# tashoyan/locations-recommender

Measured on AMD Instinct MI355X. Metric: KNN person-pair cosines/s (cosine place+category, combine, top-K), higher is better.
Workload: dtype u16 dot (exact, packed) / f64 cosine

## Files before the change

### locations-recommender_amd/csrc/knn.hip

```cpp

#include <algorithm>
#include <chrono>
#include <cstring>
#include <cmath>
#include <cstdlib>
#include <memory>
#include <new>
#include <numeric>
#include <type_traits>
#include <unordered_map>

#include "knn_index.h"

namespace {

using namespace locrec;

constexpr uint32_t kEmpty = 0xFFFFFFFFu;
constexpr int kMergeCap = 8192;
constexpr int kAggCap = 4096;
constexpr int kDirectMaxBytes = cfg::kDirectMaxBytes;
constexpr int kLdsSoftLimit = 64 * 1024;
constexpr int kLdsHardLimit = 160 * 1024;

// ... 406 lines not shown
    p.mode = 3;
    p.qt = ht.qt;
    p.waves = ht.waves;
    p.S = std::max(64, pow2ceil(2 * K));
    auto fam = [&](const DevFamily &d, const DevBuf<uint32_t> &sell, const DevBuf<int64_t> &off, const DevBuf<int32_t> &w,
                   Family &f) {
        f = Family{};
        f.sell = sell.p;
        f.sell_off = off.p;
        f.sell_w = w.p;
        f.norm = d.norm.p;
        f.inorm32 = d.inorm32.p;
        f.csr_ptr = d.csr_ptr.p;
        f.csr_idx = d.csr_idx.p;
        f.csr_val = d.csr_val.p;
        f.direct = 1;
    };
    fam(ix->fp, ht.p_sell, ht.p_off, ht.p_w, p.fp);
    fam(ix->fc, ht.c_sell, ht.c_off, ht.c_w, p.fc);
    p.fp.rows_cap = ht.h;
    p.fc.rows_cap = ix->fc.dim;
    size_t cur = (size_t)kHtCatRows * p.qt * 2 + (size_t)cfg::ht_plane_rows(ht.h) * p.qt * 2;
    cur = (cur + 15) & ~(size_t)15;
    p.off_tail = (int)cur;
    cur += (size_t)p.waves * 64 * p.qt * 2;
    p.off_cand_s = (int)cur;
    cur += (size_t)p.qt * p.S * sizeof(double);
    p.off_cand_rid = (int)cur;
    cur += (size_t)p.qt * p.S * sizeof(uint32_t);
    cur = (cur + 15) & ~(size_t)15;
    p.off_misc = (int)cur;
    cur += (size_t)p.qt * (3 * sizeof(double) + 8 * sizeof(int32_t)) + 16;
    cur = (cur + 15) & ~(size_t)15;
    p.off_queue = (int)cur;
    cur += (size_t)p.waves * kQueueCap * 16 + (size_t)p.waves * 4 + 16;
    p.lds = cur;
    if (cur > (size_t)kLdsHardLimit) return false;
    pl = p;
    return true;
}

int32_t enqueue_ht_prepass(locrec_knn_index *ix, const int32_t *qrows_dev, int32_t qrow0, int64_t nq, int qt,
                           int64_t total_hits)
{
    hipStream_t s = ix->stream;
    locrec::HtIndex &ht = ix->ht;
    const int ntiles = (int)((nq + qt - 1) / qt);
    const int32_t off_stride = ix->cand_slice1 - ix->cand_slice0 + 1;
    if ((size_t)total_hits + 64 > ht.hits.n) {
        int64_t want = total_hits + total_hits / 3;
        const int64_t rows = (int64_t)ht.tail_hits_ps.size() - 1;
        if (rows >= nq && nq > 0) {
            int64_t widest = 0;
            for (int64_t i = 0; i + nq <= rows; ++i) widest = std::max(widest, ht.tail_hits_ps[(size_t)(i + nq)] - ht.tail_hits_ps[(size_t)i]);
            want = qrows_dev ? std::max(widest + widest / 16, want) : std::max(widest, total_hits);
        }
        LOCREC_TRY(ht.hits.reserve((size_t)want + 64));
    }
    LOCREC_TRY(ht.off.reserve((size_t)ntiles * off_stride));
    LOCREC_TRY(ht.tile_base.reserve((size_t)ntiles + 1));
    if (!ht.err.p) {
        LOCREC_TRY(ht.err.alloc(1));
        LOCREC_HIP_TRY(hipMemsetAsync(ht.err.p, 0, sizeof(int32_t), s));
    }
    hipLaunchKernelGGL(ht_tile_bases, dim3(1), dim3(1024), 0, s, ht.tail_hits.p, qrows_dev, qrow0, (int32_t)nq, qt, ntiles,
                       ht.tile_base.p);
    HtPreParams PP{};
    PP.csr_ptr = ix->fp.csr_ptr.p;
    PP.csr_idx = ix->fp.csr_idx.p;
    PP.csr_val = ix->fp.csr_val.p;
    PP.post_ptr = ht.post_ptr.p;
    PP.post = ht.post.p;
    PP.qrows = qrows_dev;
    PP.qrow0 = qrow0;
    PP.nq = (int32_t)nq;
    PP.h = ht.h;
    PP.slice0 = ix->cand_slice0;
    PP.nslices = ix->cand_slice1;
    PP.tile_base = ht.tile_base.p;
    PP.hits = ht.hits.p;
    PP.off = ht.off.p;
    PP.off_stride = off_stride;
    PP.error = ht.err.p;
    if (qt == 32)
        hipLaunchKernelGGL(ht_build_hits<32>, dim3((unsigned)ntiles), dim3(kHtPreThreads), 0, s, PP);
    else
        hipLaunchKernelGGL(ht_build_hits<16>, dim3((unsigned)ntiles), dim3(kHtPreThreads), 0, s, PP);
    LOCREC_HIP_TRY(hipGetLastError());
    return LOCREC_OK;
}

int32_t launch_scan_ht(locrec_knn_index *ix, const Plan &pl, const ScanParams &P, dim3 grid, hipStream_t s,
                       bool seed_pass = false, bool use_seed = false, int32_t seed_stride = 1)
{
    locrec::HtIndex &ht = ix->ht;
    HtCold c{};
    size_t lds = pl.lds;
    int32_t slices_per_chunk = P.slices_per_chunk;
    if (seed_pass) {
        LOCREC_TRY(ht.seed.reserve((size_t)P.nq));
        c.seed_out = ht.seed.p;
        c.stride = seed_stride;
        slices_per_chunk = P.nslices - P.slice0;
        grid = dim3(1, grid.y);
    } else {
        c.seed = use_seed ? ht.seed.p : nullptr;
        c.stride = 1;
    }
    c.norm_p = ix->fp.norm.p;
    c.norm_c = ix->fc.norm.p;
    c.rid = P.rid;
    c.pcsr_ptr = ix->fp.csr_ptr.p;
    c.pcsr_idx = ix->fp.csr_idx.p;
    c.pcsr_val = ix->fp.csr_val.p;
    c.ccsr_ptr = ix->fc.csr_ptr.p;
    c.ccsr_idx = ix->fc.csr_idx.p;
    c.ccsr_val = ix->fc.csr_val.p;
    c.part_s = P.part_s;
    c.part_rid = P.part_rid;
    c.part_cnt = P.part_cnt;
    c.overflow = P.overflow;
    c.qrows = P.qrows;
    c.pw = P.pw;
    c.cw = P.cw;
    c.qrow0 = P.qrow0;
    c.nq = P.nq;
    c.nrows = P.nrows;
    c.K = P.K;
    c.S = P.S;
    c.h = ht.h;
    c.c_rows = ix->fc.dim;
    c.nchunks = P.nchunks;
    c.off_tail = pl.off_tail;
    c.off_cand_s = pl.off_cand_s;
    c.off_cand_rid = pl.off_cand_rid;
    c.off_misc = pl.off_misc;
    c.off_queue = pl.off_queue;
    if (seed_pass) {
        c.off_misc = pl.off_cand_s;
        c.off_hist = pl.off_cand_s + 1024;
        lds = (size_t)c.off_hist + (size_t)pl.qt * pl.waves * 64 * sizeof(uint32_t);
    }
    c.flush_mask = P.flush_mask;
    c.enter_threads = P.enter_threads;
    c.fast = P.fast;
    if (const char *e = debug_env("LOCREC_DEBUG_HT")) c.dbg = std::atoi(e);
#ifdef LOCREC_DEBUG_SWITCHES
    if (debug_env("LOCREC_DEBUG_HT_CLOCKS")) {
        static unsigned long long *dbg_dev = nullptr;
        if (!dbg_dev) {
            LOCREC_HIP_TRY(hipMalloc(reinterpret_cast<void **>(&dbg_dev), 16 * sizeof(unsigned long long)));
            LOCREC_HIP_TRY(hipMemset(dbg_dev, 0, 16 * sizeof(unsigned long long)));
        }
        unsigned long long prev[16];
        LOCREC_HIP_TRY(hipStreamSynchronize(s));
        LOCREC_HIP_TRY(hipMemcpy(prev, dbg_dev, sizeof prev, hipMemcpyDeviceToHost));
        fprintf(stderr, "[locrec ht clocks of the previous launch, summed over waves] hot %llu resolve %llu sync %llu drain %llu | slices with a passing pair %llu, resolve q-iterations %llu, sync iterations %llu, sync rounds %llu\n",
                prev[0], prev[1], prev[2], prev[3], prev[4], prev[5], prev[6], prev[7]);
        fprintf(stderr, "[locrec ht work by wave index] %llu %llu %llu %llu %llu %llu %llu %llu\n", prev[8], prev[9], prev[10], prev[11],
                prev[12], prev[13], prev[14], prev[15]);
        LOCREC_HIP_TRY(hipMemset(dbg_dev, 0, 16 * sizeof(unsigned long long)));
        c.dbg_out = dbg_dev;
    }
#endif
    LOCREC_HIP_TRY(hipMemcpyAsync(ht.cold.p, &c, sizeof c, hipMemcpyHostToDevice, s));
    auto kern = seed_pass ? knn_scan_ht<16, 8, true>
                          : pl.waves == 6 ? knn_scan_ht<16, 6> : pl.waves == 12 ? knn_scan_ht<16, 12> : knn_scan_ht<16, 8>;
    if (lds > 64 * 1024)
        LOCREC_HIP_TRY(hipFuncSetAttribute(reinterpret_cast<const void *>(kern),
                                           hipFuncAttributeMaxDynamicSharedMemorySize, (int)lds));
// ... 640 lines not shown
        hipLaunchKernelGGL(knn_pack_host, dim3(blocks), dim3(256), 0, s, a);
    }
};

void shard_slice_range(locrec_knn_index *ix, int32_t index, int32_t count, int32_t *s0, int32_t *s1)
{
    const int32_t ns = ix->nslices;
    if (ix->slice_cost.empty()) {
        ix->slice_cost.assign((size_t)ns + 1, 0);
        for (int32_t sl = 0; sl < ns; ++sl) {
            int wp = 0, wc = 0;
            for (int64_t r = (int64_t)sl * 64; r < std::min<int64_t>(ix->n, (int64_t)(sl + 1) * 64); ++r) {
                wp = std::max(wp, ix->fp.nnz[r]);
                wc = std::max(wc, ix->fc.nnz[r]);
            }
            ix->slice_cost[sl + 1] = ix->slice_cost[sl] + 64 * (int64_t)(((wp + 3) & ~3) + ((wc + 3) & ~3)) + 64;
        }
    }
    auto cut = [&](int32_t i) -> int32_t {
        if (i <= 0) return 0;
        if (i >= count) return ns;
        const int64_t want = ix->slice_cost[ns] / count * i;
        return (int32_t)(std::lower_bound(ix->slice_cost.begin(), ix->slice_cost.end(), want) - ix->slice_cost.begin());
    };
    *s0 = std::min(cut(index), ns);
    *s1 = std::min(std::max(cut(index + 1), *s0), ns);
}

struct CandRangeGuard {
    locrec_knn_index *ix;
    CandRangeGuard(locrec_knn_index *i, int32_t s0, int32_t s1) : ix(i)
    {
        ix->cand_slice0 = s0;
        ix->cand_slice1 = s1;
    }
    ~CandRangeGuard()
    {
        ix->cand_slice0 = 0;
        ix->cand_slice1 = ix->nslices;
    }
};

}

using namespace locrec;

namespace locrec {
int32_t knn_enqueue_dense(locrec_knn_index *ix, int32_t qrow, double pw, double cw)
{
    bool fits = false;
    LOCREC_TRY(enqueue_dense_impl(ix, qrow, pw, cw, &fits));
    if (!fits) return fail(LOCREC_E_INVALID_ARG, "query vector too long for the single-request scan");
    return LOCREC_OK;
}

unsigned char *knn_stage(locrec_knn_index *ix) { return stage_of(ix); }
}

namespace locrec {
void knn_read_env(locrec_knn_index *ix)
{
    ix->force_hash = std::getenv("LOCREC_KNN_FORCE_HASH") != nullptr;
    if (const char *e = std::getenv("LOCREC_KNN_QT")) ix->qt_max = std::max(1, std::atoi(e));
    ix->no_single = std::getenv("LOCREC_KNN_NO_SINGLE") != nullptr;
    ix->no_fast = std::getenv("LOCREC_KNN_NO_FAST") != nullptr;
    ix->no_dense_hash = std::getenv("LOCREC_KNN_NO_DENSE_HASH") != nullptr;
    ix->no_wide_block = std::getenv("LOCREC_KNN_NO_WIDE_BLOCK") != nullptr;
    if (const char *e = std::getenv("LOCREC_KNN_WAVES")) ix->waves16 = std::atoi(e) == 4 ? 4 : 8;
    ix->no_ht = std::getenv("LOCREC_KNN_NO_HT") != nullptr;
    ix->no_direct8 = std::getenv("LOCREC_KNN_NO_DIRECT8") != nullptr;
    ix->no_pack = std::getenv("LOCREC_KNN_NO_PACK") != nullptr;
    ix->no_seed = std::getenv("LOCREC_KNN_NO_SEED") != nullptr;
    ix->ht_round4 = std::getenv("LOCREC_KNN_HT_ROUND4") != nullptr;
    ix->no_tile_special = std::getenv("LOCREC_KNN_NO_TILE_SPECIAL") != nullptr;
    if (const char *e = std::getenv("LOCREC_KNN_SEED_MIN_SLICES")) ix->seed_min_slices = std::max(1, std::atoi(e));
    if (const char *e = std::getenv("LOCREC_KNN_SEED_SAMPLE")) ix->seed_sample_slices = std::max(8, std::atoi(e));
    ix->force_dense_query = std::getenv("LOCREC_KNN_FORCE_DENSE_QUERY") != nullptr;
    ix->ht.v1 = std::getenv("LOCREC_KNN_HT_V1") != nullptr;
    if (const char *e = std::getenv("LOCREC_KNN_HT_W")) {
        const int w = std::atoi(e);
        if (w == 6 || w == 8 || w == 12) ix->ht.waves = w;
    }
    if (ix->ht.v1) ix->ht.waves = 8;
    ix->force_generic = std::getenv("LOCREC_KNN_FORCE_GENERIC") != nullptr;
    ix->no_pack16 = std::getenv("LOCREC_KNN_NO_PACK16") != nullptr;
    ix->no_pop = std::getenv("LOCREC_KNN_NO_POP") != nullptr;
    ix->no_row_fallback = std::getenv("LOCREC_KNN_NO_ROW_FALLBACK") != nullptr;
    if (const char *e = std::getenv("LOCREC_KNN_HT_H")) ix->env_ht_h = std::max(4, std::atoi(e));
    if (const char *e = std::getenv("LOCREC_KNN_POP_H")) ix->env_pop_h = std::max(64, std::atoi(e));
    if (const char *e = std::getenv("LOCREC_KNN_BLOCKS")) ix->env_blocks = std::max(1, std::atoi(e));
    if (const char *e = std::getenv("LOCREC_KNN_FLUSH")) {
        const int v = std::atoi(e);
        if (v >= 1 && v <= 64 && (v & (v - 1)) == 0) ix->env_flush = v;
    }
    if (const char *e = std::getenv("LOCREC_KNN_ENTER")) ix->env_enter = std::max(0, std::atoi(e));
}

bool knn_host_build_requested() { return std::getenv("LOCREC_KNN_HOST_BUILD") != nullptr; }
}

#include "knn_host_build.h"

extern "C" int32_t locrec_knn_create_from_device(
    int64_t n, const int64_t *person_ids,
    const int64_t *p_rowptr, const int32_t *p_idx, const double *p_val, int32_t p_dim,
    const int64_t *c_rowptr, const int32_t *c_idx, const double *c_val, int32_t c_dim,
    const int64_t *r_rowptr, const int64_t *r_place, const int64_t *r_rating,
    locrec_knn_index **out) try
{
    return knn_build_device(n, person_ids, p_rowptr, p_idx, p_val, p_dim, c_rowptr, c_idx, c_val, c_dim, r_rowptr, r_place,
                            r_rating, out);
} LOCREC_CATCH_ALL

extern "C" int32_t locrec_knn_create(
    int64_t n, const int64_t *person_ids,
    const int64_t *p_rowptr, const int32_t *p_idx, const double *p_val, int32_t p_dim,
    const int64_t *c_rowptr, const int32_t *c_idx, const double *c_val, int32_t c_dim,
    const int64_t *r_rowptr, const int64_t *r_place, const int64_t *r_rating,
    locrec_knn_index **out) try
{
    if (locrec::knn_host_build_requested())
        return knn_create_host(n, person_ids, p_rowptr, p_idx, p_val, p_dim, c_rowptr, c_idx, c_val, c_dim, r_rowptr, r_place,
                               r_rating, out);
    if (!out) return fail(LOCREC_E_INVALID_ARG, "out_index is NULL");
    *out = nullptr;
    if (n < 0 || n >= ((int64_t)1 << 31) - 64) return fail(LOCREC_E_INVALID_ARG, "bad person count");
    if (n > 0 && (!person_ids || !p_rowptr || !c_rowptr)) return fail(LOCREC_E_INVALID_ARG, "NULL input array");
    if (p_dim <= 0 || c_dim <= 0) return fail(LOCREC_E_INVALID_ARG, "vector sizes must be positive");
    LOCREC_TRY(ensure_device());
    auto check_ptr = [&](const char *name, const int64_t *ptr) -> int32_t {
        if (!ptr || n == 0) return LOCREC_OK;
        if (ptr[0] != 0) return fail(LOCREC_E_INVALID_ARG, "%s rowptr must start at 0", name);
        for (int64_t r = 0; r < n; ++r)
            if (ptr[r + 1] < ptr[r]) return fail(LOCREC_E_INVALID_ARG, "%s rowptr not monotone at %lld", name, (long long)r);
        return LOCREC_OK;
    };
    LOCREC_TRY(check_ptr("place", p_rowptr));
    LOCREC_TRY(check_ptr("category", c_rowptr));
    LOCREC_TRY(check_ptr("ratings", r_rowptr));
    const int64_t pe = n > 0 ? p_rowptr[n] : 0, ce = n > 0 ? c_rowptr[n] : 0, re = n > 0 && r_rowptr ? r_rowptr[n] : 0;
    if ((pe > 0 && (!p_idx || !p_val)) || (ce > 0 && (!c_idx || !c_val)) || (re > 0 && (!r_place || !r_rating)))
        return fail(LOCREC_E_INVALID_ARG, "NULL input array");
    DevBuf<int64_t> d_ids, d_pp, d_cp, d_rp, d_rpl, d_rra;
    DevBuf<int32_t> d_pi, d_ci;
    DevBuf<double> d_pv, d_cv;
    LOCREC_TRY(d_ids.upload(person_ids, (size_t)n));
    LOCREC_TRY(d_pp.upload(p_rowptr, n > 0 ? (size_t)n + 1 : 0));
    LOCREC_TRY(d_pi.upload(p_idx, (size_t)pe));
    LOCREC_TRY(d_pv.upload(p_val, (size_t)pe));
    LOCREC_TRY(d_cp.upload(c_rowptr, n > 0 ? (size_t)n + 1 : 0));
    LOCREC_TRY(d_ci.upload(c_idx, (size_t)ce));
    LOCREC_TRY(d_cv.upload(c_val, (size_t)ce));
    if (r_rowptr) {
        LOCREC_TRY(d_rp.upload(r_rowptr, n > 0 ? (size_t)n + 1 : 0));
        LOCREC_TRY(d_rpl.upload(r_place, (size_t)re));
        LOCREC_TRY(d_rra.upload(r_rating, (size_t)re));
    }
    LOCREC_HIP_TRY(hipDeviceSynchronize());
    return knn_build_device(n, d_ids.p, d_pp.p, d_pi.p, d_pv.p, p_dim, d_cp.p, d_ci.p, d_cv.p, c_dim, r_rowptr ? d_rp.p : nullptr,
                            r_rowptr ? d_rpl.p : nullptr, r_rowptr ? d_rra.p : nullptr, out);
} LOCREC_CATCH_ALL

extern "C" int32_t locrec_knn_destroy(locrec_knn_index *ix) try
{
    if (!ix) return LOCREC_OK;
    (void)hipSetDevice(ix->device);
// ... 854 lines not shown
```

### locations-recommender_amd/csrc/knn_ht.h

```cpp

constexpr int kHtCatRows = 64;
constexpr int kHtMaxEntries = 1024;
constexpr int kHtSubSlices = 4096;
constexpr int kHtPreThreads = 512;


__host__ __device__ __forceinline__ uint32_t ht_pack_hit(uint32_t lane, uint32_t q, uint32_t prod)
{
    return (lane << 21) | (q << 16) | prod;
}

template <int QT>
__device__ __forceinline__ uint32_t ht_tail_word(uint32_t r, uint32_t w)
{
    constexpr uint32_t chunks = QT / 8;
    const uint32_t sw = chunks == 2 ? ((r >> 3) & 1u) : ((r >> 2) & 3u);
    return r * (QT * 2) + ((((w >> 2) ^ sw) & (chunks - 1)) << 4) + ((w & 3u) << 2);
}

struct HtPreParams {
    const int64_t *csr_ptr;
    const int32_t *csr_idx;
    const double *csr_val;
    const int64_t *post_ptr;
    const uint32_t *post;
    const int32_t *qrows;
    int32_t qrow0, nq;
    int32_t h;
    int32_t slice0, nslices;
    const int64_t *tile_base;
    uint32_t *hits;
    uint32_t *off;
    int32_t off_stride;
    int32_t *error;
};

__global__ __launch_bounds__(1024) void ht_tile_bases(const int64_t *tail_hits, const int32_t *qrows, int32_t qrow0,
                                                      int32_t nq, int32_t qt, int32_t ntiles, int64_t *tile_base)
{
    __shared__ int64_t wsum[16];
    __shared__ int64_t carry;
    const int tid = threadIdx.x, lane = tid & 63, wave = tid >> 6;
    if (tid == 0) carry = 0;
    __syncthreads();
    for (int t0 = 0; t0 < ntiles; t0 += 1024) {
        const int t = t0 + tid;
        int64_t mine = 0;
        if (t < ntiles)
            for (int q = t * qt; q < min(nq, (t + 1) * qt); ++q) mine += tail_hits[qrows ? qrows[q] : qrow0 + q];
        int64_t inc = mine;
#pragma unroll
        for (int d = 1; d < 64; d <<= 1) {
            const int64_t o = __shfl_up(inc, d);
            if (lane >= d) inc += o;
        }
        if (lane == 63) wsum[wave] = inc;
        __syncthreads();
        int64_t before = carry;
        for (int w = 0; w < wave; ++w) before += wsum[w];
        if (t < ntiles) tile_base[t] = before + inc - mine;
        __syncthreads();
        if (tid == 1023) carry = before + inc;
        __syncthreads();
    }
    if (tid == 0) tile_base[ntiles] = carry;
}

template <int QT>
__global__ __launch_bounds__(kHtPreThreads) void ht_build_hits(const HtPreParams P)
{
    __shared__ int64_t e_cur[kHtMaxEntries];
    __shared__ int64_t e_end[kHtMaxEntries];
    __shared__ uint32_t e_qv[kHtMaxEntries];
    __shared__ uint32_t cnt[kHtSubSlices];
    __shared__ uint32_t wtot[kHtPreThreads / 64 + 1];
    __shared__ int s_ne;
    const int tid = threadIdx.x, lane = tid & 63;
    const int wave = __builtin_amdgcn_readfirstlane(tid >> 6);
    constexpr int NW = kHtPreThreads / 64;
    const int tile = blockIdx.x;
    const int q0 = tile * QT;
    const int nqt = min(QT, P.nq - q0);
    if (tid == 0) s_ne = 0;
    __syncthreads();
    for (int q = 0; q < nqt; ++q) {
        const int row = P.qrows ? P.qrows[q0 + q] : P.qrow0 + q0 + q;
        for (int64_t e = P.csr_ptr[row] + tid; e < P.csr_ptr[row + 1]; e += kHtPreThreads) {
            const int idx = P.csr_idx[e];
            if (idx >= P.h) {
                const int slot = atomicAdd(&s_ne, 1);
                if (slot < kHtMaxEntries) {
                    const int64_t b = P.post_ptr[idx - P.h];
                    e_cur[slot] = b;
                    e_end[slot] = P.post_ptr[idx - P.h + 1];
                    e_qv[slot] = ((uint32_t)q << 16) | (uint32_t)P.csr_val[e];
                }
            }
        }
    }
    __syncthreads();
    const int ne = min(s_ne, kHtMaxEntries);
    if (s_ne > kHtMaxEntries && tid == 0 && P.error) atomicAdd(P.error, 1);
    if (P.slice0 > 0) {
        const uint32_t first_row = (uint32_t)P.slice0 * 64u;
        for (int e = tid; e < ne; e += kHtPreThreads) {
            int64_t a = e_cur[e], b = e_end[e];
            while (a < b) {
                const int64_t m = (a + b) >> 1;
                if ((P.post[m] >> 8) < first_row) a = m + 1; else b = m;
            }
            e_cur[e] = a;
        }
        __syncthreads();
    }
    uint32_t *off_row = P.off + (int64_t)tile * P.off_stride;
    uint32_t *hits = P.hits + P.tile_base[tile];
    uint32_t run = 0;
    for (int sl0 = P.slice0; sl0 < P.nslices; sl0 += kHtSubSlices) {
        const int nsl = min(kHtSubSlices, P.nslices - sl0);
        const uint32_t row_end = (uint32_t)(sl0 + nsl) * 64u;
        for (int i = tid; i < nsl; i += kHtPreThreads) cnt[i] = 0u;
        __syncthreads();
        for (int e = wave; e < ne; e += NW) {
            const int64_t end = e_end[e];
            for (int64_t p = e_cur[e]; p < end; p += 64) {
                const bool in = p + lane < end;
                const uint32_t row = in ? (P.post[p + lane] >> 8) : 0xFFFFFFFFu;
                const bool mine = in && row < row_end;
                if (mine) atomicAdd(&cnt[(row >> 6) - sl0], 1u);
                if (!__all(mine)) break;
            }
        }
        __syncthreads();
        constexpr int PER = kHtSubSlices / kHtPreThreads;
        uint32_t local[PER];
        uint32_t sum = 0;
#pragma unroll
        for (int j = 0; j < PER; ++j) {
            const int i = tid * PER + j;
            local[j] = i < nsl ? cnt[i] : 0u;
            sum += local[j];
        }
        uint32_t inc = sum;
#pragma unroll
        for (int d = 1; d < 64; d <<= 1) {
            const uint32_t o = __shfl_up(inc, d);
            if (lane >= d) inc += o;
        }
        if (lane == 63) wtot[wave] = inc;
        __syncthreads();
        if (tid == 0) {
            uint32_t acc = 0;
            for (int w = 0; w < NW; ++w) {
                const uint32_t t = wtot[w];
                wtot[w] = acc;
                acc += t;
            }
            wtot[NW] = acc;
        }
        __syncthreads();
        uint32_t excl = run + wtot[wave] + inc - sum;
        const uint32_t total = wtot[NW];
#pragma unroll
        for (int j = 0; j < PER; ++j) {
            const int i = tid * PER + j;
            if (i < nsl) {
                cnt[i] = excl;
                off_row[(sl0 - P.slice0) + i] = excl;
            }
            excl += local[j];
        }
        __syncthreads();
        for (int e = wave; e < ne; e += NW) {
            const int64_t end = e_end[e];
            const uint32_t qv = e_qv[e];
            const uint32_t q = qv >> 16, qval = qv & 0xFFFFu;
            int64_t p = e_cur[e];
            for (; p < end; p += 64) {
                const bool in = p + lane < end;
                const uint32_t pv = in ? P.post[p + lane] : 0xFFFFFFFFu;
                const uint32_t row = pv >> 8;
                const bool mine = in && row < row_end;
                if (mine) {
                    const uint32_t pos = atomicAdd(&cnt[(row >> 6) - sl0], 1u);
                    hits[pos] = ht_pack_hit(row & 63u, q, (pv & 0xFFu) * qval);
                }
                const uint64_t m = __ballot(mine);
                if (m != ~0ull) {
                    p += __popcll(m);
                    break;
                }
            }
            if (lane == 0) e_cur[e] = p < end ? p : end;
        }
        run += total;
        __syncthreads();
    }
    if (tid == 0) off_row[P.nslices - P.slice0] = run;
}


template <int QT>
__device__ void ht_build_panel(const Family &f, int rows, int plane_rows, const int *s_qrow, int nqt, unsigned short *panel)
{
    const int tid = threadIdx.x;
    uint32_t *p32 = reinterpret_cast<uint32_t *>(panel);
    for (int i = tid; i < plane_rows * QT / 2; i += blockDim.x) p32[i] = 0u;
    __syncthreads();
    for (int q = 0; q < nqt; ++q) {
        const int row = s_qrow[q];
        unsigned short *plane = panel + (q >> 3) * plane_rows * 8 + (q & 7);
        for (int64_t e = f.csr_ptr[row] + tid; e < f.csr_ptr[row + 1]; e += blockDim.x) {
            const int idx = f.csr_idx[e];
            if (idx < rows) plane[idx * 8] = (unsigned short)f.csr_val[e];
        }
    }
    __syncthreads();
}

template <int QT>
__device__ __forceinline__ void ht_accum4(const u32x4 e4, const unsigned char *panel, int stride, uint32_t (&acc)[QT / 2])
{
    const uint32_t ee[4] = {e4.x, e4.y, e4.z, e4.w};
#pragma unroll
    for (int t = 0; t < 4; ++t) {
        const unsigned char *r = panel + (ee[t] & 0xFFFFu);
#pragma unroll
        for (int i = 0; i < QT / 8; ++i) {
            const u32x4 pv = *reinterpret_cast<const u32x4 *>(r + i * stride);
            asm("v_pk_mad_u16 %0, %1, %2, %0 op_sel:[0,1,0]" : "+v"(acc[4 * i + 0]) : "v"(pv.x), "v"(ee[t]));
            asm("v_pk_mad_u16 %0, %1, %2, %0 op_sel:[0,1,0]" : "+v"(acc[4 * i + 1]) : "v"(pv.y), "v"(ee[t]));
            asm("v_pk_mad_u16 %0, %1, %2, %0 op_sel:[0,1,0]" : "+v"(acc[4 * i + 2]) : "v"(pv.z), "v"(ee[t]));
            asm("v_pk_mad_u16 %0, %1, %2, %0 op_sel:[0,1,0]" : "+v"(acc[4 * i + 3]) : "v"(pv.w), "v"(ee[t]));
        }
    }
}

template <int QT>
__device__ __forceinline__ void ht_family_dots(const unsigned char *panel, int stride, const u32x4 *lane_base, int w4, Group4 cur,
                                               uint32_t (&acc)[QT / 2])
{
    for (int j = 0; j < w4; j += 4) {
        const Group4 nxt = load_group(lane_base, j + 4, w4);
        ht_accum4<QT>(cur.a0, panel, stride, acc);
        if (j + 1 < w4) ht_accum4<QT>(cur.a1, panel, stride, acc);
        if (j + 2 < w4) ht_accum4<QT>(cur.a2, panel, stride, acc);
        if (j + 3 < w4) ht_accum4<QT>(cur.a3, panel, stride, acc);
        cur = nxt;
    }
}


struct HtSliceDesc {
    uint32_t off_p4;
    uint32_t off_c4;
    uint32_t w4;
    uint32_t cnt;
};

struct HtCold {
    const double *norm_p, *norm_c;
    const uint32_t *rid;
    const int64_t *pcsr_ptr;
    const int32_t *pcsr_idx;
    const double *pcsr_val;
    const int64_t *ccsr_ptr;
    const int32_t *ccsr_idx;
    const double *ccsr_val;
    double *part_s;
    uint32_t *part_rid;
    int32_t *part_cnt;
    int32_t *overflow;
    const int32_t *qrows;
    double pw, cw;
    int32_t qrow0, nq, nrows, K, S, h, c_rows, nchunks;
    int32_t off_tail, off_cand_s, off_cand_rid, off_misc, off_queue;
    int32_t flush_mask, enter_threads, fast;
    const double *seed;
    double *seed_out;
    int32_t stride, off_hist;
    unsigned long long *dbg_out;
    int32_t dbg;
// ... 613 lines not shown
```

### locations-recommender_amd/csrc/knn_index.h

```cpp
#pragma once

#include <algorithm>

#include "common.h"

namespace locrec {

namespace cfg {
constexpr int kDirectMaxBytes = 16384;
constexpr int kPopTable = 4096;
constexpr int kHtQt = 16;
constexpr int kHtHead = 512;
__host__ __device__ constexpr int ht_plane_rows(int h) { return h > kHtHead ? h : kHtHead; }
constexpr int kHtCatRows = 64;
constexpr int kHtNP = 4;
constexpr int kHtColdBytes = 512;
}

struct DevFamily {
    DevBuf<uint32_t> sell;
    DevBuf<double> sell_val;
    DevBuf<int64_t> sell_off;
    DevBuf<int32_t> sell_w;
    DevBuf<double> norm;
    DevBuf<float> inorm32;
    DevBuf<int64_t> csr_ptr;
    DevBuf<int32_t> csr_idx;
    DevBuf<double> csr_val;
    int32_t dim = 0, vbits = 0;
    int64_t scan_bytes = 0;
    std::vector<int32_t> nnz;
    DevBuf<int32_t> sell_split;
    int32_t pop_h = 0;
};


struct HtIndex {
    bool ready = false;
    int32_t h = 0;
    int32_t qt = 16;
    int32_t waves = 8;
    DevBuf<uint32_t> p_sell, c_sell;
    DevBuf<int64_t> p_off, c_off;
    DevBuf<int32_t> p_w, c_w;
    DevBuf<int64_t> post_ptr;
    DevBuf<uint32_t> post;
    DevBuf<uint4> desc;
    int64_t mult_words = 0;
    std::vector<uint32_t> slice_cnt;
    DevBuf<uint32_t> rid;
    DevBuf<uint32_t> ss;
    DevBuf<unsigned char> cold;
    DevBuf<double> seed;
    bool v1 = false;
    DevBuf<int64_t> tail_hits;
    std::vector<int64_t> tail_hits_ps;
    std::vector<int32_t> tail_nnz;
    int64_t scan_bytes = 0;
    DevBuf<uint32_t> hits, off;
    DevBuf<int64_t> tile_base;
    DevBuf<int32_t> err;
};

}

using locrec::DevBuf;
using locrec::DevFamily;
using locrec::KernelProfile;

struct locrec_knn_index {
    int device = 0;
    hipStream_t stream = nullptr;
    bool own_stream = false;
    int64_t n = 0;
    int32_t nslices = 0;
    int32_t cand_slice0 = 0, cand_slice1 = 0;
    std::vector<int64_t> slice_cost;
    bool packed = false;
    bool pack16 = false;
    bool force_hash = false;
    bool no_wide_block = false;
    bool no_dense_hash = false;
    int qt_max = 16;
    int waves16 = 8;
    DevFamily fp, fc;
    locrec::HtIndex ht;
    bool no_ht = false;
    DevBuf<uint32_t> rid;
    DevBuf<int64_t> ids_by_rank;
    DevBuf<int32_t> row_of_rid;
    DevBuf<int64_t> r_ptr, r_place;
    DevBuf<double> r_rating;
    int64_t max_r_nnz = 0;
    DevBuf<int32_t> r_pidx;
    DevBuf<int64_t> cplace_dev;
    DevBuf<int64_t> cp_ptr;
    DevBuf<int32_t> cp_row;
    DevBuf<double> cp_rating;
    std::vector<int64_t> cplace_ids;
    DevBuf<uint64_t> lk_keys, lk_keys_out;
    DevBuf<uint32_t> lk_vals, lk_vals_out;
    DevBuf<unsigned char> lk_temp;
    DevBuf<double> lk_w, lk_ws, lk_ss;
    DevBuf<int64_t> lk_out_place, lk_out_n;
    DevBuf<double> lk_out_est;
    DevBuf<int32_t> lk_tile_cnt;
    DevBuf<int64_t> lk_seg_begin, lk_seg_end;
    DevBuf<int32_t> lk_place_seg0;
    DevBuf<double> lk_seg_ws, lk_seg_ss;
    int32_t lk_nsegs = -1;
    DevBuf<double> lkb_S, lkb_qd_p, lkb_qd_c, lkb_seg_ws, lkb_seg_ss, lkb_ws, lkb_ss, lkb_est;
    DevBuf<int32_t> lkb_cand, lkb_tile_cnt;
    DevBuf<int64_t> lkb_place;
    std::vector<int64_t> lkb_off;
    bool have_lkb = false;
    bool lkb_deferred = false;
    std::vector<int32_t> wide_rows;
    std::vector<unsigned char> is_wide;
    DevBuf<int32_t> wide_rows_dev;
    DevBuf<int2> side_p, side_c;
    DevBuf<int32_t> side_off_p, side_off_c, side_w_p, side_w_c;
    bool row_is_wide(int32_t r) const { return !is_wide.empty() && is_wide[(size_t)r] != 0; }
    std::vector<int64_t> ids_row;
    std::vector<int32_t> row_of_input;
    std::vector<int64_t> ids_sorted;
    std::vector<int32_t> row_by_rank;
    int32_t row_of_person(int64_t id) const
    {
        const auto it = std::lower_bound(ids_sorted.begin(), ids_sorted.end(), id);
        return it == ids_sorted.end() || *it != id ? -1 : row_by_rank[(size_t)(it - ids_sorted.begin())];
    }
    DevBuf<int32_t> qrows;
    DevBuf<int32_t> qrows_patch;
    std::vector<int32_t> qrows_host;
    DevBuf<double> part_s;
    DevBuf<uint32_t> part_rid;
    DevBuf<int32_t> part_cnt;
// ... 102 lines not shown
```

Measured before the change: 1015 billion.

## Stage HT prepass hits in LDS with adaptive slice width and coalesced writes

Replaces the two-pass count-then-scatter prepass that builds the hit lists with a single-pass variant. Each slice window's hits are gathered into a dynamic LDS stage using ballot/mbcnt compaction, counting-sorted by slice in LDS, then written to global memory as aligned 16-byte vector stores. The window width and lanes per posting entry are chosen per tile from the expected hit density, and cursors shrink to 32 bits. The aim is to avoid rereading postings twice and to replace scattered global writes. It falls back to the two-pass path when the stage overflows, adding complexity and LDS pressure.

Result: faster. 1035 billion, median of 6 (+2.0%).

```diff
diff --git a/locations-recommender_amd/csrc/knn.hip b/locations-recommender_amd/csrc/knn.hip
--- a/locations-recommender_amd/csrc/knn.hip
+++ b/locations-recommender_amd/csrc/knn.hip
@@ -512,10 +512,23 @@
     PP.off = ht.off.p;
     PP.off_stride = off_stride;
     PP.error = ht.err.p;
-    if (qt == 32)
-        hipLaunchKernelGGL(ht_build_hits<32>, dim3((unsigned)ntiles), dim3(kHtPreThreads), 0, s, PP);
-    else
-        hipLaunchKernelGGL(ht_build_hits<16>, dim3((unsigned)ntiles), dim3(kHtPreThreads), 0, s, PP);
+    PP.stage = ht.pre_stage > 0 ? ht.pre_stage : kHtPreStageDefault;
+    if (ht.pre_v1 || ht.post.n + 64 > 0xFFFFFFFFull) {
+        if (qt == 32)
+            hipLaunchKernelGGL(ht_build_hits_v1<32>, dim3((unsigned)ntiles), dim3(kHtPreThreads), 0, s, PP);
+        else
+            hipLaunchKernelGGL(ht_build_hits_v1<16>, dim3((unsigned)ntiles), dim3(kHtPreThreads), 0, s, PP);
+    } else {
+        const size_t lds = ht_pre_stage_bytes(PP.stage);
+        const dim3 grid((unsigned)ntiles), block(kHtPreThreads);
+        if (qt == 32) {
+            if (PP.stage <= kHtPreStageSmall) hipLaunchKernelGGL((ht_build_hits<32, 8>), grid, block, lds, s, PP);
+            else hipLaunchKernelGGL((ht_build_hits<32, 16>), grid, block, lds, s, PP);
+        } else {
+            if (PP.stage <= kHtPreStageSmall) hipLaunchKernelGGL((ht_build_hits<16, 8>), grid, block, lds, s, PP);
+            else hipLaunchKernelGGL((ht_build_hits<16, 16>), grid, block, lds, s, PP);
+        }
+    }
     LOCREC_HIP_TRY(hipGetLastError());
     return LOCREC_OK;
 }
@@ -1322,6 +1335,9 @@
         if (w == 6 || w == 8 || w == 12) ix->ht.waves = w;
     }
     if (ix->ht.v1) ix->ht.waves = 8;
+    ix->ht.pre_v1 = std::getenv("LOCREC_KNN_HT_PRE_V1") != nullptr;
+    if (const char *e = std::getenv("LOCREC_KNN_HT_PRE_STAGE"))
+        ix->ht.pre_stage = std::min(kHtPreStageMax, std::max(kHtPreStageMin, std::atoi(e)));
     ix->force_generic = std::getenv("LOCREC_KNN_FORCE_GENERIC") != nullptr;
     ix->no_pack16 = std::getenv("LOCREC_KNN_NO_PACK16") != nullptr;
     ix->no_pop = std::getenv("LOCREC_KNN_NO_POP") != nullptr;
diff --git a/locations-recommender_amd/csrc/knn_ht.h b/locations-recommender_amd/csrc/knn_ht.h
--- a/locations-recommender_amd/csrc/knn_ht.h
+++ b/locations-recommender_amd/csrc/knn_ht.h
@@ -1,14 +1,9 @@
 
 constexpr int kHtCatRows = 64;
-constexpr int kHtMaxEntries = 1024;
-constexpr int kHtSubSlices = 4096;
-constexpr int kHtPreThreads = 512;
-
-
-__host__ __device__ __forceinline__ uint32_t ht_pack_hit(uint32_t lane, uint32_t q, uint32_t prod)
-{
-    return (lane << 21) | (q << 16) | prod;
-}
+
+
+#include "knn_ht_prepass.h"
+
 
 template <int QT>
 __device__ __forceinline__ uint32_t ht_tail_word(uint32_t r, uint32_t w)
@@ -18,186 +13,6 @@
     return r * (QT * 2) + ((((w >> 2) ^ sw) & (chunks - 1)) << 4) + ((w & 3u) << 2);
 }
 
-struct HtPreParams {
-    const int64_t *csr_ptr;
-    const int32_t *csr_idx;
-    const double *csr_val;
-    const int64_t *post_ptr;
-    const uint32_t *post;
-    const int32_t *qrows;
-    int32_t qrow0, nq;
-    int32_t h;
-    int32_t slice0, nslices;
-    const int64_t *tile_base;
-    uint32_t *hits;
-    uint32_t *off;
-    int32_t off_stride;
-    int32_t *error;
-};
-
-__global__ __launch_bounds__(1024) void ht_tile_bases(const int64_t *tail_hits, const int32_t *qrows, int32_t qrow0,
-                                                      int32_t nq, int32_t qt, int32_t ntiles, int64_t *tile_base)
-{
-    __shared__ int64_t wsum[16];
-    __shared__ int64_t carry;
-    const int tid = threadIdx.x, lane = tid & 63, wave = tid >> 6;
-    if (tid == 0) carry = 0;
-    __syncthreads();
-    for (int t0 = 0; t0 < ntiles; t0 += 1024) {
-        const int t = t0 + tid;
-        int64_t mine = 0;
-        if (t < ntiles)
-            for (int q = t * qt; q < min(nq, (t + 1) * qt); ++q) mine += tail_hits[qrows ? qrows[q] : qrow0 + q];
-        int64_t inc = mine;
-#pragma unroll
-        for (int d = 1; d < 64; d <<= 1) {
-            const int64_t o = __shfl_up(inc, d);
-            if (lane >= d) inc += o;
-        }
-        if (lane == 63) wsum[wave] = inc;
-        __syncthreads();
-        int64_t before = carry;
-        for (int w = 0; w < wave; ++w) before += wsum[w];
-        if (t < ntiles) tile_base[t] = before + inc - mine;
-        __syncthreads();
-        if (tid == 1023) carry = before + inc;
-        __syncthreads();
-    }
-    if (tid == 0) tile_base[ntiles] = carry;
-}
-
-template <int QT>
-__global__ __launch_bounds__(kHtPreThreads) void ht_build_hits(const HtPreParams P)
-{
-    __shared__ int64_t e_cur[kHtMaxEntries];
-    __shared__ int64_t e_end[kHtMaxEntries];
-    __shared__ uint32_t e_qv[kHtMaxEntries];
-    __shared__ uint32_t cnt[kHtSubSlices];
-    __shared__ uint32_t wtot[kHtPreThreads / 64 + 1];
-    __shared__ int s_ne;
-    const int tid = threadIdx.x, lane = tid & 63;
-    const int wave = __builtin_amdgcn_readfirstlane(tid >> 6);
-    constexpr int NW = kHtPreThreads / 64;
-    const int tile = blockIdx.x;
-    const int q0 = tile * QT;
-    const int nqt = min(QT, P.nq - q0);
-    if (tid == 0) s_ne = 0;
-    __syncthreads();
-    for (int q = 0; q < nqt; ++q) {
-        const int row = P.qrows ? P.qrows[q0 + q] : P.qrow0 + q0 + q;
-        for (int64_t e = P.csr_ptr[row] + tid; e < P.csr_ptr[row + 1]; e += kHtPreThreads) {
-            const int idx = P.csr_idx[e];
-            if (idx >= P.h) {
-                const int slot = atomicAdd(&s_ne, 1);
-                if (slot < kHtMaxEntries) {
-                    const int64_t b = P.post_ptr[idx - P.h];
-                    e_cur[slot] = b;
-                    e_end[slot] = P.post_ptr[idx - P.h + 1];
-                    e_qv[slot] = ((uint32_t)q << 16) | (uint32_t)P.csr_val[e];
-                }
-            }
-        }
-    }
-    __syncthreads();
-    const int ne = min(s_ne, kHtMaxEntries);
-    if (s_ne > kHtMaxEntries && tid == 0 && P.error) atomicAdd(P.error, 1);
-    if (P.slice0 > 0) {
-        const uint32_t first_row = (uint32_t)P.slice0 * 64u;
-        for (int e = tid; e < ne; e += kHtPreThreads) {
-            int64_t a = e_cur[e], b = e_end[e];
-            while (a < b) {
-                const int64_t m = (a + b) >> 1;
-                if ((P.post[m] >> 8) < first_row) a = m + 1; else b = m;
-            }
-            e_cur[e] = a;
-        }
-        __syncthreads();
-    }
-    uint32_t *off_row = P.off + (int64_t)tile * P.off_stride;
-    uint32_t *hits = P.hits + P.tile_base[tile];
-    uint32_t run = 0;
-    for (int sl0 = P.slice0; sl0 < P.nslices; sl0 += kHtSubSlices) {
-        const int nsl = min(kHtSubSlices, P.nslices - sl0);
-        const uint32_t row_end = (uint32_t)(sl0 + nsl) * 64u;
-        for (int i = tid; i < nsl; i += kHtPreThreads) cnt[i] = 0u;
-        __syncthreads();
-        for (int e = wave; e < ne; e += NW) {
-            const int64_t end = e_end[e];
-            for (int64_t p = e_cur[e]; p < end; p += 64) {
-                const bool in = p + lane < end;
-                const uint32_t row = in ? (P.post[p + lane] >> 8) : 0xFFFFFFFFu;
-                const bool mine = in && row < row_end;
-                if (mine) atomicAdd(&cnt[(row >> 6) - sl0], 1u);
-                if (!__all(mine)) break;
-            }
-        }
-        __syncthreads();
-        constexpr int PER = kHtSubSlices / kHtPreThreads;
-        uint32_t local[PER];
-        uint32_t sum = 0;
-#pragma unroll
-        for (int j = 0; j < PER; ++j) {
-            const int i = tid * PER + j;
-            local[j] = i < nsl ? cnt[i] : 0u;
-            sum += local[j];
-        }
-        uint32_t inc = sum;
-#pragma unroll
-        for (int d = 1; d < 64; d <<= 1) {
-            const uint32_t o = __shfl_up(inc, d);
-            if (lane >= d) inc += o;
-        }
-        if (lane == 63) wtot[wave] = inc;
-        __syncthreads();
-        if (tid == 0) {
-            uint32_t acc = 0;
-            for (int w = 0; w < NW; ++w) {
-                const uint32_t t = wtot[w];
-                wtot[w] = acc;
-                acc += t;
-            }
-            wtot[NW] = acc;
-        }
-        __syncthreads();
-        uint32_t excl = run + wtot[wave] + inc - sum;
-        const uint32_t total = wtot[NW];
-#pragma unroll
-        for (int j = 0; j < PER; ++j) {
-            const int i = tid * PER + j;
-            if (i < nsl) {
-                cnt[i] = excl;
-                off_row[(sl0 - P.slice0) + i] = excl;
-            }
-            excl += local[j];
-        }
-        __syncthreads();
-        for (int e = wave; e < ne; e += NW) {
-            const int64_t end = e_end[e];
-            const uint32_t qv = e_qv[e];
-            const uint32_t q = qv >> 16, qval = qv & 0xFFFFu;
-            int64_t p = e_cur[e];
-            for (; p < end; p += 64) {
-                const bool in = p + lane < end;
-                const uint32_t pv = in ? P.post[p + lane] : 0xFFFFFFFFu;
-                const uint32_t row = pv >> 8;
-                const bool mine = in && row < row_end;
-                if (mine) {
-                    const uint32_t pos = atomicAdd(&cnt[(row >> 6) - sl0], 1u);
-                    hits[pos] = ht_pack_hit(row & 63u, q, (pv & 0xFFu) * qval);
-                }
-                const uint64_t m = __ballot(mine);
-                if (m != ~0ull) {
-                    p += __popcll(m);
-                    break;
-                }
-            }
-            if (lane == 0) e_cur[e] = p < end ? p : end;
-        }
-        run += total;
-        __syncthreads();
-    }
-    if (tid == 0) off_row[P.nslices - P.slice0] = run;
-}
 
 
 template <int QT>
diff --git a/locations-recommender_amd/csrc/knn_ht_prepass.h b/locations-recommender_amd/csrc/knn_ht_prepass.h
--- /dev/null
+++ b/locations-recommender_amd/csrc/knn_ht_prepass.h
@@ -0,0 +1,372 @@
+
+constexpr int kHtMaxEntries = 1024;
+constexpr int kHtSubSlices = 4096;
+constexpr int kHtPreThreads = 512;
+constexpr int kHtPreWidthMax = 512;
+constexpr int kHtPreStageMax = 8192;
+constexpr int kHtPreStageSmall = 4096;
+constexpr int kHtPreStageDefault = 8192;
+constexpr int kHtPreStageMin = 64;
+static_assert(kHtPreWidthMax == kHtPreThreads, "the staged form's prefix gives every thread one slice");
+
+__host__ __device__ __forceinline__ uint32_t ht_pack_hit(uint32_t lane, uint32_t q, uint32_t prod)
+{
+    return (lane << 21) | (q << 16) | prod;
+}
+
+struct HtPreParams {
+    const int64_t *csr_ptr;
+    const int32_t *csr_idx;
+    const double *csr_val;
+    const int64_t *post_ptr;
+    const uint32_t *post;
+    const int32_t *qrows;
+    int32_t qrow0, nq;
+    int32_t h;
+    int32_t slice0, nslices;
+    const int64_t *tile_base;
+    uint32_t *hits;
+    uint32_t *off;
+    int32_t off_stride;
+    int32_t *error;
+    int32_t stage;
+};
+
+inline size_t ht_pre_stage_bytes(int stage) { return ((size_t)stage + 4) * 4 + (size_t)stage * 2; }
+
+__global__ __launch_bounds__(1024) void ht_tile_bases(const int64_t *tail_hits, const int32_t *qrows, int32_t qrow0,
+                                                      int32_t nq, int32_t qt, int32_t ntiles, int64_t *tile_base)
+{
+    __shared__ int64_t wsum[16];
+    __shared__ int64_t carry;
+    const int tid = threadIdx.x, lane = tid & 63, wave = tid >> 6;
+    if (tid == 0) carry = 0;
+    __syncthreads();
+    for (int t0 = 0; t0 < ntiles; t0 += 1024) {
+        const int t = t0 + tid;
+        int64_t mine = 0;
+        if (t < ntiles)
+            for (int q = t * qt; q < min(nq, (t + 1) * qt); ++q) mine += tail_hits[qrows ? qrows[q] : qrow0 + q];
+        int64_t inc = mine;
+#pragma unroll
+        for (int d = 1; d < 64; d <<= 1) {
+            const int64_t o = __shfl_up(inc, d);
+            if (lane >= d) inc += o;
+        }
+        if (lane == 63) wsum[wave] = inc;
+        __syncthreads();
+        int64_t before = carry;
+        for (int w = 0; w < wave; ++w) before += wsum[w];
+        if (t < ntiles) tile_base[t] = before + inc - mine;
+        __syncthreads();
+        if (tid == 1023) carry = before + inc;
+        __syncthreads();
+    }
+    if (tid == 0) tile_base[ntiles] = carry;
+}
+
+template <class CUR>
+__device__ int ht_pre_entries(const HtPreParams &P, int q0, int nqt, int first_slice, CUR *e_cur, CUR *e_end, uint32_t *e_qv,
+                              int *s_ne)
+{
+    const int tid = threadIdx.x;
+    if (tid == 0) *s_ne = 0;
+    __syncthreads();
+    for (int q = 0; q < nqt; ++q) {
+        const int row = P.qrows ? P.qrows[q0 + q] : P.qrow0 + q0 + q;
+        for (int64_t e = P.csr_ptr[row] + tid; e < P.csr_ptr[row + 1]; e += kHtPreThreads) {
+            const int idx = P.csr_idx[e];
+            if (idx >= P.h) {
+                const int slot = atomicAdd(s_ne, 1);
+                if (slot < kHtMaxEntries) {
+                    e_cur[slot] = (CUR)P.post_ptr[idx - P.h];
+                    e_end[slot] = (CUR)P.post_ptr[idx - P.h + 1];
+                    e_qv[slot] = ((uint32_t)q << 16) | (uint32_t)P.csr_val[e];
+                }
+            }
+        }
+    }
+    __syncthreads();
+    const int ne = min(*s_ne, kHtMaxEntries);
+    if (*s_ne > kHtMaxEntries && tid == 0 && P.error) atomicAdd(P.error, 1);
+    if (first_slice > 0) {
+        const uint32_t first_row = (uint32_t)first_slice * 64u;
+        for (int e = tid; e < ne; e += kHtPreThreads) {
+            CUR a = e_cur[e], b = e_end[e];
+            while (a < b) {
+                const CUR m = a + ((b - a) >> 1);
+                if ((P.post[m] >> 8) < first_row) a = m + 1; else b = m;
+            }
+            e_cur[e] = a;
+        }
+        __syncthreads();
+    }
+    return ne;
+}
+
+template <class CUR, int CAP>
+__device__ uint32_t ht_pre_two_pass(const HtPreParams &P, int ne, CUR *e_cur, const CUR *e_end, const uint32_t *e_qv,
+                                    uint32_t *cnt, uint32_t *wtot, int sl0, int nsl, uint32_t run, uint32_t *off_row,
+                                    uint32_t *hits)
+{
+    static_assert(CAP % kHtPreThreads == 0, "every thread owns CAP / threads consecutive counters");
+    constexpr int NW = kHtPreThreads / 64;
+    const int tid = threadIdx.x, lane = tid & 63;
+    const int wave = __builtin_amdgcn_readfirstlane(tid >> 6);
+    const uint32_t row_end = (uint32_t)(sl0 + nsl) * 64u;
+    for (int i = tid; i < nsl; i += kHtPreThreads) cnt[i] = 0u;
+    __syncthreads();
+    for (int e = wave; e < ne; e += NW) {
+        const CUR end = e_end[e];
+        for (CUR p = e_cur[e]; p < end; p += 64) {
+            const bool in = p + lane < end;
+            const uint32_t row = in ? (P.post[p + lane] >> 8) : 0xFFFFFFFFu;
+            const bool mine = in && row < row_end;
+            if (mine) atomicAdd(&cnt[(row >> 6) - sl0], 1u);
+            if (!__all(mine)) break;
+        }
+    }
+    __syncthreads();
+    constexpr int PER = CAP / kHtPreThreads;
+    uint32_t local[PER];
+    uint32_t sum = 0;
+#pragma unroll
+    for (int j = 0; j < PER; ++j) {
+        const int i = tid * PER + j;
+        local[j] = i < nsl ? cnt[i] : 0u;
+        sum += local[j];
+    }
+    uint32_t inc = sum;
+#pragma unroll
+    for (int d = 1; d < 64; d <<= 1) {
+        const uint32_t o = __shfl_up(inc, d);
+        if (lane >= d) inc += o;
+    }
+    if (lane == 63) wtot[wave] = inc;
+    __syncthreads();
+    if (tid == 0) {
+        uint32_t acc = 0;
+        for (int w = 0; w < NW; ++w) {
+            const uint32_t t = wtot[w];
+            wtot[w] = acc;
+            acc += t;
+        }
+        wtot[NW] = acc;
+    }
+    __syncthreads();
+    uint32_t excl = run + wtot[wave] + inc - sum;
+    const uint32_t total = wtot[NW];
+#pragma unroll
+    for (int j = 0; j < PER; ++j) {
+        const int i = tid * PER + j;
+        if (i < nsl) {
+            cnt[i] = excl;
+            off_row[(sl0 - P.slice0) + i] = excl;
+        }
+        excl += local[j];
+    }
+    __syncthreads();
+    for (int e = wave; e < ne; e += NW) {
+        const CUR end = e_end[e];
+        const uint32_t qv = e_qv[e];
+        const uint32_t q = qv >> 16, qval = qv & 0xFFFFu;
+        CUR p = e_cur[e];
+        for (; p < end; p += 64) {
+            const bool in = p + lane < end;
+            const uint32_t pv = in ? P.post[p + lane] : 0xFFFFFFFFu;
+            const uint32_t row = pv >> 8;
+            const bool mine = in && row < row_end;
+            if (mine) {
+                const uint32_t pos = atomicAdd(&cnt[(row >> 6) - sl0], 1u);
+                hits[pos] = ht_pack_hit(row & 63u, q, (pv & 0xFFu) * qval);
+            }
+            const uint64_t m = __ballot(mine);
+            if (m != ~0ull) {
+                p += __popcll(m);
+                break;
+            }
+        }
+        if (lane == 0) e_cur[e] = p < end ? p : end;
+    }
+    __syncthreads();
+    return total;
+}
+
+template <int QT>
+__global__ __launch_bounds__(kHtPreThreads) void ht_build_hits_v1(const HtPreParams P)
+{
+    __shared__ int64_t e_cur[kHtMaxEntries];
+    __shared__ int64_t e_end[kHtMaxEntries];
+    __shared__ uint32_t e_qv[kHtMaxEntries];
+    __shared__ uint32_t cnt[kHtSubSlices];
+    __shared__ uint32_t wtot[kHtPreThreads / 64 + 1];
+    __shared__ int s_ne;
+    const int tile = blockIdx.x;
+    const int q0 = tile * QT;
+    const int ne = ht_pre_entries<int64_t>(P, q0, min(QT, P.nq - q0), P.slice0, e_cur, e_end, e_qv, &s_ne);
+    uint32_t *off_row = P.off + (int64_t)tile * P.off_stride;
+    uint32_t *hits = P.hits + P.tile_base[tile];
+    uint32_t run = 0;
+    for (int sl0 = P.slice0; sl0 < P.nslices; sl0 += kHtSubSlices)
+        run += ht_pre_two_pass<int64_t, kHtSubSlices>(P, ne, e_cur, e_end, e_qv, cnt, wtot, sl0, min(kHtSubSlices, P.nslices - sl0),
+                                                      run, off_row, hits);
+    if (threadIdx.x == 0) off_row[P.nslices - P.slice0] = run;
+}
+
+
+constexpr int kHtPreBatches = 8;
+
+template <int QT, int RECS>
+__global__ __launch_bounds__(kHtPreThreads, RECS == 8 ? 8 : 4) void ht_build_hits(const HtPreParams P)
+{
+    extern __shared__ __align__(16) unsigned char ht_pre_smem[];
+    __shared__ uint32_t e_cur[kHtMaxEntries];
+    __shared__ uint32_t e_end[kHtMaxEntries];
+    __shared__ uint32_t e_qv[kHtMaxEntries];
+    __shared__ uint32_t cnt[kHtPreWidthMax];
+    __shared__ uint32_t wtot[kHtPreThreads / 64 + 1];
+    __shared__ int s_ne;
+    __shared__ uint32_t s_n;
+    constexpr int NW = kHtPreThreads / 64, NB = kHtPreBatches;
+    const int stage = P.stage;
+    uint32_t *st_hit = reinterpret_cast<uint32_t *>(ht_pre_smem);
+    unsigned short *st_sl = reinterpret_cast<unsigned short *>(st_hit + stage + 4);
+    const int tid = threadIdx.x, lane = tid & 63;
+    const int wave = __builtin_amdgcn_readfirstlane(tid >> 6);
+    const int tile = blockIdx.x;
+    const int q0 = tile * QT;
+    const int nqt = min(QT, P.nq - q0);
+    int ne = ht_pre_entries<uint32_t>(P, q0, nqt, P.slice0, e_cur, e_end, e_qv, &s_ne);
+    uint32_t *off_row = P.off + (int64_t)tile * P.off_stride;
+    const int64_t tbase = P.tile_base[tile];
+    uint32_t *hits = P.hits + tbase;
+    int width = 1, seg_log = 2;
+    {
+        const int64_t tot = P.tile_base[tile + 1] - tbase;
+        const int64_t all = P.nslices - P.slice0;
+        const int64_t target = (int64_t)(stage / 2) * all / (tot > 0 ? tot : 1);
+        while (width < kHtPreWidthMax && (int64_t)width * 10 <= target * 7) width *= 2;
+        const int64_t per_entry2 = 2 * tot * width / (all * (ne > 0 ? ne : 1));
+        while (seg_log < 6 && (1 << seg_log) < per_entry2) ++seg_log;
+    }
+    const int seg_lanes = 1 << seg_log;
+    const int seg = lane >> seg_log;
+    const uint32_t k = (uint32_t)lane & (uint32_t)(seg_lanes - 1);
+    const uint64_t seg_mask = (seg_lanes == 64 ? ~0ull : ((1ull << seg_lanes) - 1ull)) << (seg << seg_log);
+    const int per_step = 64 >> seg_log;
+    const int nsteps = (ne + per_step - 1) / per_step;
+    uint32_t run = 0;
+    for (int sl0 = P.slice0; sl0 < P.nslices; sl0 += width) {
+        const int nsl = min(width, P.nslices - sl0);
+        const uint32_t row0 = (uint32_t)sl0 * 64u, row_end = (uint32_t)(sl0 + nsl) * 64u;
+        const uint32_t mis = (uint32_t)((tbase + run) & 3);
+        if (tid < nsl) cnt[tid] = 0u;
+        if (tid == 0) s_n = 0u;
+        __syncthreads();
+        for (int s0 = wave; s0 < nsteps; s0 += NW * NB) {
+            uint32_t c[NB], en[NB], pv[NB];
+            bool act[NB], in[NB];
+#pragma unroll
+            for (int j = 0; j < NB; ++j) {
+                const int e = (s0 + j * NW) * per_step + seg;
+                act[j] = s0 + j * NW < nsteps && e < ne;
+                c[j] = act[j] ? e_cur[e] : 0u;
+                en[j] = act[j] ? e_end[e] : 0u;
+            }
+            bool again;
+            do {
+#pragma unroll
+                for (int j = 0; j < NB; ++j) {
+                    in[j] = act[j] && k < en[j] - c[j];
+                    pv[j] = in[j] ? P.post[c[j] + k] : 0u;
+                }
+                uint64_t m[NB];
+                uint32_t before[NB], total = 0;
+#pragma unroll
+                for (int j = 0; j < NB; ++j) {
+                    m[j] = __ballot(in[j] && (pv[j] >> 8) < row_end);
+                    before[j] = total;
+                    total += (uint32_t)__popcll(m[j]);
+                }
+                again = false;
+                if (total != 0u) {
+                    uint32_t at = 0;
+                    if (lane == 0) at = atomicAdd(&s_n, total);
+                    const uint32_t base = (uint32_t)__builtin_amdgcn_readfirstlane(at);
+#pragma unroll
+                    for (int j = 0; j < NB; ++j) {
+                        const uint32_t row = pv[j] >> 8;
+                        const uint32_t pos = base + before[j] +
+                                             __builtin_amdgcn_mbcnt_hi((uint32_t)(m[j] >> 32), __builtin_amdgcn_mbcnt_lo((uint32_t)m[j], 0u));
+                        if (((m[j] >> lane) & 1ull) && pos < (uint32_t)stage) {
+                            const uint32_t qv = e_qv[(s0 + j * NW) * per_step + seg];
+                            st_hit[mis + pos] = ht_pack_hit(row & 63u, qv >> 16, (pv[j] & 0xFFu) * (qv & 0xFFFFu));
+                            st_sl[pos] = (unsigned short)((row - row0) >> 6);
+                        }
+                        const uint32_t took = (uint32_t)__popcll(m[j] & seg_mask);
+                        c[j] += took;
+                        act[j] = took == (uint32_t)seg_lanes && c[j] < en[j];
+                        if (k == 0u && took > 0u) e_cur[(s0 + j * NW) * per_step + seg] = c[j];
+                        again = again || act[j];
+                    }
+                }
+            } while (__any(again));
+        }
+        __syncthreads();
+        const uint32_t n = s_n;
+        if (n > (uint32_t)stage) {
+            ne = ht_pre_entries<uint32_t>(P, q0, nqt, sl0, e_cur, e_end, e_qv, &s_ne);
+            run += ht_pre_two_pass<uint32_t, kHtPreWidthMax>(P, ne, e_cur, e_end, e_qv, cnt, wtot, sl0, nsl, run, off_row, hits);
+            continue;
+        }
+        if (n == 0u) {
+            if (tid < nsl) off_row[(sl0 - P.slice0) + tid] = run;
+            continue;
+        }
+        uint32_t rec_hit[RECS];
+#pragma unroll
+        for (int r = 0; r < RECS; ++r) {
+            const uint32_t i = (uint32_t)(tid + r * kHtPreThreads);
+            if (i < n) {
+                rec_hit[r] = st_hit[mis + i];
+                atomicAdd(&cnt[st_sl[i]], 1u);
+            }
+        }
+        __syncthreads();
+        const uint32_t mine = tid < nsl ? cnt[tid] : 0u;
+        uint32_t inc = mine;
+#pragma unroll
+        for (int d = 1; d < 64; d <<= 1) {
+            const uint32_t o = __shfl_up(inc, d);
+            if (lane >= d) inc += o;
+        }
+        if (lane == 63) wtot[wave] = inc;
+        __syncthreads();
+        uint32_t excl = inc - mine;
+        for (int w = 0; w < wave; ++w) excl += wtot[w];
+        if (tid < nsl) {
+            cnt[tid] = excl;
+            off_row[(sl0 - P.slice0) + tid] = run + excl;
+        }
+        __syncthreads();
+#pragma unroll
+        for (int r = 0; r < RECS; ++r) {
+            const uint32_t i = (uint32_t)(tid + r * kHtPreThreads);
+            if (i < n) st_hit[mis + atomicAdd(&cnt[st_sl[i]], 1u)] = rec_hit[r];
+        }
+        __syncthreads();
+        {
+            uint32_t *dst = hits + run - mis;
+            const uint32_t last = mis + n;
+            for (uint32_t g = (uint32_t)tid * 4u; g < last; g += kHtPreThreads * 4u) {
+                if (g >= mis && g + 4u <= last) {
+                    *reinterpret_cast<u32x4 *>(dst + g) = *reinterpret_cast<const u32x4 *>(st_hit + g);
+                } else {
+                    for (uint32_t i = max(g, mis); i < min(g + 4u, last); ++i) dst[i] = st_hit[i];
+                }
+            }
+        }
+        run += n;
+    }
+    if (tid == 0) off_row[P.nslices - P.slice0] = run;
+}
diff --git a/locations-recommender_amd/csrc/knn_index.h b/locations-recommender_amd/csrc/knn_index.h
--- a/locations-recommender_amd/csrc/knn_index.h
+++ b/locations-recommender_amd/csrc/knn_index.h
@@ -53,6 +53,8 @@
     DevBuf<unsigned char> cold;
     DevBuf<double> seed;
     bool v1 = false;
+    bool pre_v1 = false;
+    int32_t pre_stage = 0;
     DevBuf<int64_t> tail_hits;
     std::vector<int64_t> tail_hits_ps;
     std::vector<int32_t> tail_nnz;
```
